# xiph/daala

Hardware: NVIDIA H100
Metric: encoder Mpixels/s on 4K YUV420 intra (higher is better)
Workload: dtype int32

## Files before the change

daala_b200/csrc/kf_engine.cu:

```cuda
#include <cuda_runtime.h>
#include <math.h>
#include <stdint.h>
#include <stdio.h>
#include <stdlib.h>
#include <string.h>

#include <algorithm>
#include <cmath>
#include <mutex>
#include <new>
#include <vector>

#include "daala_b200.h"
#include "dering_search.h"
#include "late_skip.h"
#include "lossless.h"
#include "mc_batch.h"
#include "gen/coding_order.inc"
#include "pvq_math.cuh"
#include "pvq_warp.cuh"
#include "pvq_common.cuh"

namespace daala_b200 {
namespace kf {

using namespace daala_b200::pvq;

enum Cnt {
  kNLuma = 0, kNChroma, kLumaCoefs, kChromaCoefs,
  kNItemsL = 4,
  kNItemsC = 7,
  kTotalHi = 14,
  kNHeads = 15,
  kNHeads0 = 16,
  kError = 17,
  kDepsDone = 18,
  kMcBadRef = 19,
  kMcBeyond = 20,
  kHeadLoL = 32,
  kHeadLoC = 64,
  kHeadHi = 96,
  kTailHi = 128,
  kDoneHi = 160,
  kHeadCh = 192,
  kWaiters = 224,
  kTraceN = 240,
  kCntWords = 256
};

constexpr int kTile = 1024;
constexpr int kMaxLevels = 4096;
constexpr int kLevelBins = kMaxLevels * 3;

struct Lists {
  const uint8_t* bsize;
  int bstride;
  long long bsize_pitch;
  int F, UW, UH;
  int u_row0, u_rows;
  int ntiles;
  int4* tile_sum;
  int32_t* unit_lbase;
  int32_t* unit_loff;
  daala_b200_pvq_block* luma;
  daala_b200_pvq_block* chroma;
  int32_t* dep_top;
  int32_t* dep_left;
  int32_t* succ_bottom;
  int32_t* succ_right;
  uint32_t* items_l[3];
  uint32_t* items_c[3];
  uint32_t* heads;
  uint32_t* heads0;
// ... 570 lines not shown
  }
  return kNoItem;
}

__device__ __forceinline__ void intra_band_ref(const Stage& S, int blk, int band, int coef_off, int lane) {
  const daala_b200_pvq_params& prm = S.prm;
  const int start = band_start(band);
  const int bn = band_start(band + 1) - start;
  const int r = band % 3;
  int top = -1, left = -1;
  if (band == 0 || r == 1) top = S.dep_top[blk];
  if (band == 0 || r == 2) left = S.dep_left[blk];
  if (band == 3 || band == 6) top = left = -1;
  const int32_t* ot = top >= 0 ? prm.out + prm.blocks[top].coef_off : nullptr;
  const int32_t* ol = left >= 0 ? prm.out + prm.blocks[left].coef_off : nullptr;
  bool low_from_top = false;
  if (band == 0) {
    double g1 = 0, g2 = 0;
    if (ot) { double a = __ldcg(ot + 2), bb = __ldcg(ot + 5), c = __ldcg(ot + 9); g1 += a * a; g1 += bb * bb; g1 += c * c; }
    if (ol) { double a = __ldcg(ol + 1), bb = __ldcg(ol + 4), c = __ldcg(ol + 7); g2 += a * a; g2 += bb * bb; g2 += c * c; }
    low_from_top = g1 > g2;
  }
  int32_t* vref = prm.ref + coef_off;
  for (int i = start + lane; i < start + bn; i += 32) {
    int r2, c2;
    scan_rc(i, &r2, &c2);
    int32_t p = 0;
    if (r2 == 0 && c2 > 0 && ot && (c2 >= 4 || low_from_top)) p = __ldcg(ot + i);
    if (c2 == 0 && r2 > 0 && ol && (r2 >= 4 || !low_from_top)) p = __ldcg(ol + i);
    vref[i] = p;
  }
}

template <bool kIntra>
__device__ __forceinline__ void run_item(const Stage& S, uint32_t item, int lane, int16_t* snap) {
  const daala_b200_pvq_params& prm = S.prm;
  const int blk = (int)(item >> 4), band = (int)(item & 15);
  const daala_b200_pvq_block b = prm.blocks[blk];
  const int bs = b.bs, pli = b.pli;
  const int start = band_start(band);
  const int bn = band_start(band + 1) - start;
  const size_t off = (size_t)b.coef_off + start;
  if (kIntra) intra_band_ref(S, blk, band, b.coef_off, lane);
  int qidx = bs * (bs + 1) + (band + 1) - (band + 1) / 3;
  int q = (prm.q0 * prm.pvq_qm_q4[pli][qidx]) >> 4;
  if (q < 1) q = 1;
  const int beta = (prm.use_masking && pli == 0 && bs > 0) ? kBeta15 : kBeta1;
  const int qoff = (b.xdec & 1 ? prm.qm_stride : 0) + ((((1 << (2 * bs)) - 1) << 4) / 3) + start;
  int itheta, max_theta, k;
  double skip_term;
  const bool pre = kIntra && S.pre_ev && band != 3 && band != 6;
  const int32_t* pev = pre ? S.pre_ev + (off >> 3) * kPreEvWords : nullptr;
  const int16_t* psn = pre ? S.pre_snap + 2 * off : nullptr;
  const int gain = quantise_band_warp<0>(lane, snap, S.rsqrt_tbl, prm.out + off, prm.in + off, prm.ref + off, bn, q,
                                         prm.y + off, &itheta, &max_theta, &k, beta, &skip_term, prm.is_keyframe, pli,
                                         prm.qm + qoff, prm.qm_inv + qoff, prm.pvq_norm_lambda, pev, psn);
  if (lane == 0) {
    const size_t r = (size_t)blk * 9 + band;
    prm.res_skip_term[r] = skip_term;
    short4 pk;
    pk.x = (short)gain; pk.y = (short)itheta; pk.z = (short)max_theta; pk.w = (short)k;
    reinterpret_cast<short4*>(S.res_pack)[r] = pk;
  }
}

struct ItemGeom {
  int blk, band, bn, q, beta, pli, qoff;
  size_t off;
};
__device__ __forceinline__ int band_q(const daala_b200_pvq_params& prm, const daala_b200_kf_frame_quant* fq, int frame,
                                      int pli, int qidx) {
  return fq ? (fq[frame].q0 * fq[frame].pvq_qm_q4[pli][qidx]) >> 4 : (prm.q0 * prm.pvq_qm_q4[pli][qidx]) >> 4;
}
__device__ __forceinline__ ItemGeom item_geom(const daala_b200_pvq_params& prm, uint32_t item,
                                              const daala_b200_kf_frame_quant* fq) {
  ItemGeom g;
  g.blk = (int)(item >> 4);
  g.band = (int)(item & 15);
  const daala_b200_pvq_block b = prm.blocks[g.blk];
  const int bs = b.bs;
  g.pli = b.pli;
  const int start = band_start(g.band);
  g.bn = band_start(g.band + 1) - start;
  g.off = (size_t)b.coef_off + start;
  const int qidx = bs * (bs + 1) + (g.band + 1) - (g.band + 1) / 3;
  int q = band_q(prm, fq, b.frame, g.pli, qidx);
  g.q = q < 1 ? 1 : q;
  g.beta = (prm.use_masking && g.pli == 0 && bs > 0) ? kBeta15 : kBeta1;
  g.qoff = (b.xdec & 1 ? prm.qm_stride : 0) + ((((1 << (2 * bs)) - 1) << 4) / 3) + start;
  return g;
}

template <int kPhase, bool kZeroRef, int kMode, bool kFq = false>
__global__ void __launch_bounds__(128) k_pvq_split(const __grid_constant__ Stage S, int cls, int chunk) {
  const daala_b200_pvq_params& prm = S.prm;
// ... 154 lines not shown
      if (lane == 0) {
        const int blk = (int)(item >> 4);
        if (band == 0) {
          const int nb[2] = {S.succ_bottom[blk], S.succ_right[blk]};
          for (int i = 0; i < 2; i++) {
            if (nb[i] < 0) continue;
            const int need = (S.dep_top[nb[i]] >= 0) + (S.dep_left[nb[i]] >= 0);
            if (need == 2 && atomicAdd(&S.join0[nb[i]], 1) != 1) continue;
            if (next == kNoItem) {
              next = (uint32_t)nb[i] << 4;
            } else {
              __threadfence();
              push_chain(S, nb[i], 0);
            }
          }
        } else {
          const int nb = band % 3 == 1 ? S.succ_bottom[blk] : S.succ_right[blk];
          if (nb >= 0) next = ((uint32_t)nb << 4) | band;
        }
      }
      next = __shfl_sync(0xffffffffu, next, 0);
      if (next == kNoItem) break;
      __threadfence();
      item = next;
    }
  }
}

__global__ void k_fill_rsqrt(double* tbl) {
  const int i = blockIdx.x * blockDim.x + threadIdx.x;
  if (i < kTableDoubles) pvq_fill_rsqrt_table(tbl, i);
}

enum { kBeginLuma = 1, kBeginChroma = 2 };
__global__ void k_begin_pvq(int32_t* cnt, int stages) {
  if (threadIdx.x == 0 && blockIdx.x == 0) {
    if (stages & kBeginLuma) {
      cnt[kHeadLoL] = 0;
      cnt[kHeadHi] = 0;
      cnt[kTailHi] = cnt[kNHeads0];
      cnt[kDoneHi] = 0;
      cnt[kHeadCh] = 0;
      cnt[kWaiters] = 0;
#ifdef DAALA_B200_CHAIN_TRACE
      cnt[kTraceN] = 0;
#endif
    }
    if (stages & kBeginChroma) cnt[kHeadLoC] = 0;
  }
}

template <bool kInter>
__global__ void __launch_bounds__(256) k_finish_scatter(const __grid_constant__ Stage S) {
  const daala_b200_pvq_params& prm = S.prm;
  const int n = min(S.cnt[S.n_blocks_at], S.max_blocks);
  const int lane = threadIdx.x & 31;
  const int nwarps = (gridDim.x * blockDim.x) >> 5;
  for (int blk = (blockIdx.x * blockDim.x + threadIdx.x) >> 5; blk < n; blk += nwarps) {
    const daala_b200_pvq_block b = prm.blocks[blk];
    const int ln = b.bs + 2, nn = 1 << ln;
    const int len = ln >= 5 ? 512 : 1 << (2 * ln);
    const int stride = prm.plane_stride[b.pli];
    int32_t* dst = prm.coef_plane[b.pli] + b.frame * prm.plane_frame_pitch[b.pli] + (size_t)b.y0 * stride + b.x0;
    const int32_t* src = prm.out + b.coef_off;
    if (lane == 0) {
      const int nb = num_bands(b.bs);
      double sd = 0;
      for (int i = 0; i < nb; i++) sd += prm.res_skip_term[(size_t)blk * 9 + i];
      prm.res_skip_diff[blk] = sd;
      if (!kInter) {
        prm.out[b.coef_off] = prm.in[b.coef_off];
      } else {
        int dc_quant = band_q(prm, S.fq, b.frame, b.pli, b.bs * (b.bs + 1));
        if (dc_quant < 1) dc_quant = 1;
        const int32_t r = prm.ref[b.coef_off], diff = prm.in[b.coef_off] - r;
        int qdc = 0;
        if (abs(diff) >= dc_quant * 141 / 256) {
          const int half = ((dc_quant + 1) >> 1) - 1;
          qdc = (diff + (diff < 0 ? -half : half)) / dc_quant;
        }
        prm.out[b.coef_off] = dst[0] = qdc * dc_quant + r;
// ... 467 lines not shown
  int32_t* thr[2];
  int32_t* dir;
  bool search;
  daala_b200_dering_search_batch sb;
};

enum { kEvLists, kEvForward, kEvLumaBands, kEvLumaScatter, kEvChroma, kNumEvents };

struct daala_b200_kf {
  daala_b200_kf_config cfg;
  int nhsb, nvsb, F;
  int plane_w[3], plane_h[3];
  cudaStream_t stream;
  bool own_stream;
  cudaStream_t side;
  cudaEvent_t ev[kNumEvents];
  cudaGraph_t graph;
  cudaGraphExec_t exec;
  bool captured;
  uint8_t* pixels[3];
  int32_t* coeffs[3];
  int32_t* lapped[3];
  uint8_t* pixels_out[3];
  uint8_t* pred_pixels[3];
  int32_t* pred_coeffs[3];
  uint8_t* bsize;
  int16_t *qm, *qm_inv;
  double* rsqrt_tbl;
  int16_t* sp_vec[3];
  int32_t* sp_lanes[3];
  int32_t* sp_uni[3];
  int16_t* sp_snap[3];
  int sp_slots[3];
  int16_t* lv_vec;
  int32_t* lv_lanes;
  int32_t* lv_uni;
  int16_t* lv_snap;
  int32_t* lv_bar;
  int lvl_slots, lvl_grid;
  Dering dering;
  Lists lists;
  Stage luma, chroma;
  Sym sym;
  daala_b200_frame frame;
  daala_b200_frame frame_pred;
  uint8_t* ref_pixels[3];
  int32_t* ref_slot;
  daala_b200_mv_pt* mv_grid;
  int32_t* ref_slot_next;
  int32_t* mv1_grid;
  uint32_t* mc_leaves;
  int32_t* mc_nleaves;
  daala_b200_mc_batch mc;
  uint8_t* fin_skip[2];
  int32_t* fin_dc[2];
  int32_t* dc_resid[2];
  int32_t* fin_coeffs[3];
  uint8_t* fin_pixels[3];
  uint8_t* fin_bskip[3];
  uint8_t *fin_level, *fin_coded;
  Fin fin;
  cudaGraph_t fin_graph;
  cudaGraphExec_t fin_exec;
  bool fin_captured;
  int fin_dc_limit;
  daala_b200_kf_frame_quant* fq;
// ... 185 lines not shown
    KF_CHECK(dalloc(kf, &L.items_l[c], cap_l[c]));
    KF_CHECK(dalloc(kf, &L.items_c[c], cap_c[c]));
  }
  if (kf->cfg.split_free > 0 || inter) {
    const int slots[3] = {1 << 19, 1 << 19, 3 << 15};
    for (int c = 0; c < 3; c++) {
      const int vs = c == 2 ? 128 : 32;
      kf->sp_slots[c] = slots[c];
      KF_CHECK(dalloc(kf, &kf->sp_vec[c], (size_t)slots[c] * 3 * vs));
      KF_CHECK(dalloc(kf, &kf->sp_lanes[c], (size_t)slots[c] * kCtxLaneWords * 16));
      KF_CHECK(dalloc(kf, &kf->sp_uni[c], (size_t)slots[c] * kCtxUniWords));
      KF_CHECK(dalloc(kf, &kf->sp_snap[c], (size_t)slots[c] * kMaxEvents * vs));
    }
  }
  if (kf->cfg.level_chains) {
    KF_CHECK(dalloc(kf, &L.lvl_hist, (size_t)kLevelBins));
    KF_CHECK(dalloc(kf, &L.lvl_cursor, (size_t)kLevelBins));
    KF_CHECK(dalloc(kf, &L.lvl_items, kf->chain_cap));
    L.nlevels = (kf->plane_w[0] + L.u_rows * 8) / 4 + 2;
    if (L.nlevels >= kMaxLevels) return (int)cudaErrorInvalidValue;
    kf->lvl_slots = 2048 * F;
    KF_CHECK(dalloc(kf, &kf->lv_vec, (size_t)kf->lvl_slots * 3 * 128));
    KF_CHECK(dalloc(kf, &kf->lv_lanes, (size_t)kf->lvl_slots * kCtxLaneWords * 16));
    KF_CHECK(dalloc(kf, &kf->lv_uni, (size_t)kf->lvl_slots * kCtxUniWords));
    KF_CHECK(dalloc(kf, &kf->lv_snap, (size_t)kf->lvl_slots * kMaxEvents * 128));
    KF_CHECK(dalloc(kf, &kf->lv_bar, (size_t)32));
    int per_sm = 0;
    KF_CHECK(cudaOccupancyMaxActiveBlocksPerMultiprocessor(&per_sm, k_pvq_levels, 128, 0));
    if (per_sm < 1) return (int)cudaErrorLaunchOutOfResources;
    kf->lvl_grid = per_sm * kf->sms;
  }
  {
    const int want = kf->cfg.persist_ctas_per_sm > 0 ? kf->cfg.persist_ctas_per_sm : kPersistCtas;
    int per_sm[2] = {0, 0};
    KF_CHECK(cudaFuncSetAttribute(k_pvq_persist<true>, cudaFuncAttributePreferredSharedMemoryCarveout,
                                  cudaSharedmemCarveoutMaxShared));
    KF_CHECK(cudaFuncSetAttribute(k_pvq_persist<false>, cudaFuncAttributePreferredSharedMemoryCarveout,
                                  cudaSharedmemCarveoutMaxShared));
    KF_CHECK(cudaOccupancyMaxActiveBlocksPerMultiprocessor(&per_sm[0], k_pvq_persist<true>, kPersistThreads, 0));
    KF_CHECK(cudaOccupancyMaxActiveBlocksPerMultiprocessor(&per_sm[1], k_pvq_persist<false>, kPersistThreads, 0));
    if (per_sm[0] < want || per_sm[1] < want) {
      snprintf(kf->err, sizeof(kf->err), "k_pvq_persist: %d / %d CTAs per SM resident, %d wanted", per_sm[0],
               per_sm[1], want);
      return (int)cudaErrorLaunchOutOfResources;
    }
  }
  KF_CHECK(dalloc(kf, &L.heads, inter ? 0 : kf->chain_cap));
  KF_CHECK(dalloc(kf, &L.heads_raw, inter ? 0 : kf->chain_cap));
  KF_CHECK(dalloc(kf, &L.head_bin, inter ? 0 : kf->chain_cap));
  KF_CHECK(dalloc(kf, &L.head_hist, inter ? 0 : (size_t)kLevelBins));
  KF_CHECK(dalloc(kf, &L.head_cursor, inter ? 0 : (size_t)kLevelBins));
  KF_CHECK(dalloc(kf, &L.heads0, ndep));
  KF_CHECK(dalloc(kf, &L.cnt, (size_t)kCntWords));
  kf->mc.bad_ref = L.cnt + kMcBadRef;
  kf->mc.beyond = L.cnt + kMcBeyond;

  auto setup_stage = [&](Stage& S, bool chroma) -> int {
    memset(&S, 0, sizeof(S));
    daala_b200_pvq_params& p = S.prm;
    const size_t ncoef = chroma ? luma_shard_px / 2 + 1024 : luma_shard_px + 1024;
    const size_t nblk = chroma ? L.max_chroma : L.max_luma;
    p.blocks = chroma ? L.chroma : L.luma;
    KF_CHECK(dalloc(kf, &p.in, ncoef));
    KF_CHECK(dalloc(kf, &p.ref, ncoef));
    KF_CHECK(dalloc(kf, &p.out, ncoef));
    KF_CHECK(dalloc(kf, &p.y, ncoef));
    KF_CHECK(dalloc(kf, &p.y16, ncoef));
    KF_CHECK(dalloc(kf, &p.res_skip_term, nblk * 9));
    KF_CHECK(dalloc(kf, &p.res_skip_diff, nblk));
    KF_CHECK(dalloc(kf, &p.res_flip, nblk));
    KF_CHECK(dalloc(kf, &S.res_pack, nblk * 9 * 4));
    p.res_gain = p.res_theta = p.res_max_theta = p.res_k = nullptr;
    p.res_dc = nullptr;
    if (inter) KF_CHECK(dalloc(kf, &p.res_dc, nblk));
    p.qm = kf->qm;
    p.qm_inv = kf->qm_inv;
    for (int i = 0; i < 3; i++) {
      p.coef_plane[i] = kf->coeffs[i];
// ... 8 lines not shown
    p.pvq_norm_lambda = kf->cfg.pvq_norm_lambda;
    memcpy(p.pvq_qm_q4, kf->cfg.pvq_qm_q4, sizeof(p.pvq_qm_q4));
    S.fq = kf->fq;
    for (int c = 0; c < 3; c++) S.items[c] = chroma ? L.items_c[c] : L.items_l[c];
    S.cnt = L.cnt;
    S.rsqrt_tbl = kf->rsqrt_tbl;
    for (int c = 0; c < 3; c++) {
      S.sp_vec[c] = kf->sp_vec[c];
      S.sp_lanes[c] = kf->sp_lanes[c];
      S.sp_uni[c] = kf->sp_uni[c];
      S.sp_snap[c] = kf->sp_snap[c];
      S.sp_slots[c] = kf->sp_slots[c];
      const size_t cap = chroma ? cap_c[c] : cap_l[c];
      S.sp_chunks[c] = kf->sp_slots[c] > 0 ? (int)((cap + kf->sp_slots[c] - 1) / kf->sp_slots[c]) : 0;
    }
    S.skip_lo = chroma ? 0 : kf->cfg.split_free > 1;
    S.max_waiters = getenv("DAALA_B200_MAX_WAITERS") ? atoi(getenv("DAALA_B200_MAX_WAITERS")) : kf->sms * 8;
    if (!chroma && kf->cfg.noref_prepass) {
      KF_CHECK(dalloc(kf, &S.pre_ev, (ncoef / 8 + 2) * kPreEvWords));
      KF_CHECK(dalloc(kf, &S.pre_snap, 2 * ncoef));
    }
    if (!chroma) {
      S.lvl_off = L.lvl_hist;
      S.lvl_items = L.lvl_items;
      S.nlevels = L.nlevels;
      S.lvl_slots = kf->lvl_slots;
      S.lv_vec = kf->lv_vec;
      S.lv_lanes = kf->lv_lanes;
      S.lv_uni = kf->lv_uni;
      S.lv_snap = kf->lv_snap;
      S.lv_bar = kf->lv_bar;
    }
    S.n_items_at = chroma ? kNItemsC : kNItemsL;
    S.head_lo_at = chroma ? kHeadLoC : kHeadLoL;
    S.n_blocks_at = chroma ? kNChroma : kNLuma;
    S.max_blocks = (int)nblk;
#ifdef DAALA_B200_CHAIN_TRACE
    if (!chroma && !inter) {
      S.trace_cap = (int)(luma_shard_px / 16);
      KF_CHECK(dalloc(kf, &S.trace, (size_t)S.trace_cap));
    }
#endif
    if (!chroma) {
      S.dep_top = L.dep_top;
      S.dep_left = L.dep_left;
      S.succ_bottom = L.succ_bottom;
      S.succ_right = L.succ_right;
      S.heads = L.heads;
      S.heads0 = L.heads0;
      KF_CHECK(dalloc(kf, &S.ring, inter ? 0 : kf->chain_cap));
      KF_CHECK(dalloc(kf, &S.join0, ndep));
    }
    return 0;
  };
  int rc = setup_stage(kf->luma, false);
  if (rc) return rc;
  rc = setup_stage(kf->chroma, true);
  if (rc) return rc;
  if (!inter) {
    Stage& C = kf->chroma;
    C.cfl_in = kf->luma.prm.in;
    C.cfl_out = kf->luma.prm.out;
    C.cfl_loff = L.unit_loff;
  }
  (void)luma_px;
  if (kf->cfg.inter_finish || kf->cfg.symbol_stream == 2)
    for (int c = 0; c < 2; c++) {
// ... 368 lines not shown
  }
  if (!core && (phases & DAALA_B200_KF_PVQ_CHROMA) && kf->cfg.late_skip) {
    const int rc = daala_b200_late_skip_enqueue(&kf->lsb, kf->sms * 3, s);
    if (rc) return rc;
  }
  if (!core && (phases & DAALA_B200_KF_PVQ_CHROMA) && kf->cfg.symbol_stream) enqueue_sym<true>(kf->sym, wide, s);
  if (phases & DAALA_B200_KF_INVERSE) {
    int rc = daala_b200_launch_inverse(&kf->frame, 3, s);
    if (rc) return rc;
  }
  return (int)cudaGetLastError();
}

static int enqueue_lists(daala_b200_kf* kf, cudaStream_t s) {
  const Lists& L = kf->lists;
  const int wide = kf->sms * 8;
  k_unit_tile_sums<<<L.ntiles, kTile, 0, s>>>(L);
  k_tile_scan<<<1, 1024, 0, s>>>(L);
  k_unit_emit<<<L.ntiles, kTile, 0, s>>>(L);
  const size_t nl = (size_t)L.max_luma * sizeof(int32_t);
  if (cudaMemsetAsync(L.succ_bottom, 0xff, nl, s) != cudaSuccess || cudaMemsetAsync(L.succ_right, 0xff, nl, s) != cudaSuccess)
    return (int)cudaGetLastError();
  if (L.lvl_hist && cudaMemsetAsync(L.lvl_hist, 0, sizeof(int32_t) * kLevelBins, s) != cudaSuccess) return (int)cudaGetLastError();
  if (cudaMemsetAsync(L.head_hist, 0, sizeof(int32_t) * kLevelBins, s) != cudaSuccess) return (int)cudaGetLastError();
  k_luma_deps<<<wide, 256, 0, s>>>(L);
  if (L.lvl_hist) {
    k_level_scan<<<1, 1024, 0, s>>>(L);
    k_level_scatter<<<wide, 256, 0, s>>>(L);
  }
  k_chroma_items<<<wide, 256, 0, s>>>(L);
  return 0;
}

static int enqueue_luma_bands(daala_b200_kf* kf, bool core, int begin, cudaStream_t s) {
  const int wide = kf->sms * 8;
  const int persist = kf->sms * (kf->cfg.persist_ctas_per_sm > 0 ? kf->cfg.persist_ctas_per_sm : kPersistCtas);
  if (cudaMemsetAsync(kf->luma.ring, 0xff, kf->chain_cap * sizeof(uint32_t), s) != cudaSuccess ||
      cudaMemsetAsync(kf->luma.join0, 0, (size_t)kf->luma.max_blocks * sizeof(int32_t), s) != cudaSuccess)
    return (int)cudaGetLastError();
  k_begin_pvq<<<1, 32, 0, s>>>(kf->lists.cnt, begin);
  if (!core) k_gather<kGatherLuma><<<wide, 256, 0, s>>>(kf->luma);
  if (kf->cfg.split_free > 1) enqueue_split<true>(kf, kf->luma, s);
  if (kf->luma.pre_ev) {
    k_pvq_prepass<2><<<kf->sms * 16, 128, 0, s>>>(kf->luma);
    k_pvq_prepass<1><<<kf->sms * 16, 128, 0, s>>>(kf->luma);
  }
  if (kf->cfg.level_chains) {
    if (cudaMemsetAsync(kf->lv_bar, 0, sizeof(int32_t) * 32, s) != cudaSuccess) return (int)cudaGetLastError();
    k_pvq_levels<<<kf->lvl_grid, 128, 0, s>>>(kf->luma);
  } else {
    k_pvq_persist<true><<<persist, kPersistThreads, 0, s>>>(kf->luma);
  }
  return 0;
}

static void enqueue_chroma(daala_b200_kf* kf, bool core, bool begin, cudaStream_t s) {
  const int wide = kf->sms * 8;
  if (begin) k_begin_pvq<<<1, 32, 0, s>>>(kf->lists.cnt, kBeginChroma);
  if (!core) k_gather<kGatherChroma><<<wide, 256, 0, s>>>(kf->chroma);
  if (kf->cfg.split_free > 0) enqueue_split<false>(kf, kf->chroma, s);
  else k_pvq_persist<false><<<kf->sms * (kf->cfg.persist_ctas_per_sm > 0 ? kf->cfg.persist_ctas_per_sm : kPersistCtas),
                              kPersistThreads, 0, s>>>(kf->chroma);
  if (!core) k_finish_scatter<false><<<wide, 256, 0, s>>>(kf->chroma);
}

static int kf_enqueue_step_forked(daala_b200_kf* kf) {
  cudaStream_t s = kf->stream, c = kf->side;
  const daala_b200_frame& fr = kf->cfg.dering ? kf->dering.frame : kf->frame;
  auto fork = [](cudaEvent_t e, cudaStream_t from, cudaStream_t to) {
    return cudaEventRecord(e, from) == cudaSuccess && cudaStreamWaitEvent(to, e, 0) == cudaSuccess;
  };
  if (!fork(kf->ev[kEvLists], s, c)) return (int)cudaGetLastError();
  int rc = daala_b200_launch_forward(&kf->frame, 3, c);
  if (!rc) rc = enqueue_lists(kf, s);
  if (rc) return rc;
  if (!fork(kf->ev[kEvForward], c, s)) return (int)cudaGetLastError();
  rc = enqueue_luma_bands(kf, false, kBeginLuma | kBeginChroma, s);
  if (rc) return rc;
  if (!fork(kf->ev[kEvLumaBands], s, c)) return (int)cudaGetLastError();
  enqueue_chroma(kf, false, false, c);
  k_finish_scatter<false><<<kf->sms * 128, 256, 0, s>>>(kf->luma);
  if (kf->cfg.symbol_stream) {
    if (!fork(kf->ev[kEvLumaScatter], s, c)) return (int)cudaGetLastError();
    enqueue_sym<false>(kf->sym, kf->sms * 8, c);
  }
  rc = enqueue_recon(fr, 1, 2, c);
  if (!rc) rc = enqueue_recon(fr, 0, 1, s);
  if (!rc && kf->cfg.dering) rc = enqueue_dering_luma(kf, kf->dering, s);
  if (rc) return rc;
  if (!fork(kf->ev[kEvChroma], c, s)) return (int)cudaGetLastError();
  for (int p = 1; kf->cfg.dering && p < 3; p++) {
    rc = enqueue_dering_plane(kf, kf->dering, p, s);
    if (rc) return rc;
  }
  return (int)cudaGetLastError();
}

static int kf_enqueue_step_lossless(daala_b200_kf* kf, int phases) {
  if (phases != DAALA_B200_KF_ALL) {
    snprintf(kf->err, sizeof(kf->err), "a lossless step runs whole (DAALA_B200_KF_ALL)");
    return (int)cudaErrorInvalidValue;
  }
  cudaStream_t s = kf->stream;
  const int wide = kf->sms * 8;
  if (kf->cfg.inter_mc) {
    if (cudaMemsetAsync(kf->lists.cnt + kMcBadRef, 0, 2 * sizeof(int32_t), s) != cudaSuccess) return (int)cudaGetLastError();
    int rc = daala_b200_launch_mc_leaves(&kf->mc, wide, s);
    if (!rc) rc = daala_b200_launch_mc_obmc(&kf->mc, wide, s);
    if (rc) return rc;
  }
  return daala_b200_launch_lossless(&kf->ll, s);
}

static int kf_enqueue_step(daala_b200_kf* kf, int phases) {
  if (kf->cfg.lossless) return kf_enqueue_step_lossless(kf, phases);
  if (kf->cfg.inter) return kf_enqueue_step_inter(kf, phases);
  if (phases == DAALA_B200_KF_ALL) return kf_enqueue_step_forked(kf);
  cudaStream_t s = kf->stream;
  if (phases & DAALA_B200_KF_LISTS) {
    const int rc = enqueue_lists(kf, s);
    if (rc) return rc;
  }
  if (phases & DAALA_B200_KF_FORWARD) {
    const int rc = daala_b200_launch_forward(&kf->frame, 3, s);
    if (rc) return rc;
  }
  const bool core = (phases & DAALA_B200_KF_SEARCH_ONLY) != 0;
  if (phases & DAALA_B200_KF_PVQ_LUMA) {
    const int rc = enqueue_luma_bands(kf, core, kBeginLuma, s);
    if (rc) return rc;
    if (!core) k_finish_scatter<false><<<kf->sms * 8, 256, 0, s>>>(kf->luma);
  }
  if (phases & DAALA_B200_KF_PVQ_CHROMA) {
    enqueue_chroma(kf, core, true, s);
    if (!core && kf->cfg.symbol_stream) enqueue_sym<false>(kf->sym, kf->sms * 8, s);
  }
  if (phases & DAALA_B200_KF_INVERSE) {
    int rc = kf->cfg.dering ? enqueue_dering(kf, kf->dering, s) : daala_b200_launch_inverse(&kf->frame, 3, s);
    if (rc) return rc;
  }
  return (int)cudaGetLastError();
}

static int kf_enqueue_finish(daala_b200_kf* kf) {
  cudaStream_t s = kf->stream;
  const int wide = kf->sms * 8;
  if (kf->fin_form) k_fin_unstream<<<wide, 256, 0, s>>>(kf->unstream);
  if (cudaMemsetAsync(kf->fin_coded, 0, (size_t)kf->F * kf->nhsb * kf->nvsb, s) != cudaSuccess)
    return (int)cudaGetLastError();
  k_fin_patch<<<wide, 256, 0, s>>>(kf->fin);
  k_fin_skip_map<<<wide, 256, 0, s>>>(kf->fin);
  const int rc = enqueue_dering(kf, kf->dering, s);
  if (rc) return rc;
  if (kf->fin_slot_out) k_fin_pool_store<<<dim3(wide > kf->F ? wide / kf->F : 1, 3 * kf->F), 256, 0, s>>>(kf->store);
  return (int)cudaGetLastError();
}

extern "C" {

static thread_local char g_create_err[256] = "null engine";

daala_b200_kf* daala_b200_kf_create(const daala_b200_kf_config* cfg) {
  snprintf(g_create_err, sizeof(g_create_err), "daala_b200_kf_create: invalid configuration");
  if (cfg && cfg->inter_mc && (cfg->inter_mc != 1 || cfg->inter != 1)) {
    snprintf(g_create_err, sizeof(g_create_err), "daala_b200_kf_create: inter_mc is 0 or 1, and 1 requires inter = 1");
    return nullptr;
  }
// ... 121 lines not shown
  if (kf->exec) cudaGraphExecDestroy(kf->exec);
  if (kf->graph) cudaGraphDestroy(kf->graph);
  if (kf->fin_exec) cudaGraphExecDestroy(kf->fin_exec);
  if (kf->fin_graph) cudaGraphDestroy(kf->fin_graph);
  for (void* p : kf->allocs) cudaFree(p);
  for (cudaEvent_t e : kf->ev)
    if (e) cudaEventDestroy(e);
  if (kf->side) cudaStreamDestroy(kf->side);
  if (kf->own_stream) cudaStreamDestroy(kf->stream);
  delete kf;
}

const char* daala_b200_kf_error(const daala_b200_kf* kf) { return kf ? kf->err : g_create_err; }

#ifdef DAALA_B200_CHAIN_TRACE
int daala_b200_kf_chain_trace(daala_b200_kf* kf, void** recs, int* cap) {
  if (!kf || !recs || !cap) return (int)cudaErrorInvalidValue;
  *recs = kf->luma.trace;
  *cap = kf->luma.trace_cap;
  return 0;
}
#endif

int daala_b200_kf_launches_per_step(const daala_b200_kf* kf) {
  if (!kf) return 0;
  if (kf->cfg.lossless) return (kf->cfg.inter_mc ? 2 : 0) + (kf->cfg.inter ? 1 : 2);
  auto split = [](const Stage& S) { return 3 * (S.sp_chunks[0] + S.sp_chunks[1] + S.sp_chunks[2]); };
  if (kf->cfg.inter)
    return 5 + 2 + (2 + split(kf->luma)) + (2 + split(kf->chroma)) + 2 + (kf->cfg.inter_mc ? 2 : 0) +
           (kf->cfg.symbol_stream ? 8 : 0) + (kf->cfg.late_skip ? kLateSkipLaunches : 0);
  int n = 5 + (kf->cfg.level_chains ? 2 : 0);
  n += 1;
  n += 3 + 1 + (kf->cfg.split_free > 1 ? split(kf->luma) : 0) + (kf->luma.pre_ev ? 2 : 0);
  n += 2 + (kf->cfg.split_free > 0 ? split(kf->chroma) : 1);
  n += kf->cfg.dering ? dering_launches(kf->dering, 2) : 4;
  if (kf->cfg.symbol_stream) n += 8;
  return n;
}

int daala_b200_kf_device_buffers(daala_b200_kf* kf, daala_b200_kf_buffers* out) {
  if (!kf || !out) return (int)cudaErrorInvalidValue;
  memset(out, 0, sizeof(*out));
  for (int p = 0; p < 3; p++) {
    out->pixels[p] = kf->pixels[p];
    out->coeffs[p] = kf->coeffs[p];
    out->lapped[p] = kf->lapped[p];
    out->pixels_out[p] = kf->pixels_out[p];
    out->plane_w[p] = kf->plane_w[p];
    out->plane_h[p] = kf->plane_h[p];
  }
  out->bsize = kf->bsize;
  out->counts = kf->lists.cnt;
  out->luma_blocks = kf->lists.luma;
  out->chroma_blocks = kf->lists.chroma;
  out->dep_top = kf->lists.dep_top;
  out->dep_left = kf->lists.dep_left;
  for (int c = 0; c < 3; c++) {
    out->luma_items[c] = kf->lists.items_l[c];
    out->chroma_items[c] = kf->lists.items_c[c];
  }
  out->luma_heads = kf->lists.heads;
  out->luma_heads0 = kf->lists.heads0;
  out->luma_heads_raw = kf->lists.heads_raw;
  out->luma_head_bin = kf->lists.head_bin;
  out->succ_bottom = kf->lists.succ_bottom;
  out->succ_right = kf->lists.succ_right;
  out->luma_res = kf->luma.res_pack;
// ... 532 lines not shown
```

daala_b200/csrc/pvq_warp.cuh:

```cuda
#pragma once
#include <math.h>
#include <stdint.h>

#include "pvq_math.cuh"

namespace daala_b200 {
namespace pvq {

constexpr unsigned kFull = 0xffffffffu;
constexpr int kMaxEvents = 14;
constexpr int kRsqrtEntries = 1 << 16;
constexpr int kLogEntries = 1 << 12;
constexpr int kTableDoubles = kRsqrtEntries + kLogEntries;

#ifndef DAALA_B200_PVQ_EXACT_BOUND
#define DAALA_B200_PVQ_EXACT_BOUND 4503599627370496.
#endif
#ifdef DAALA_B200_EMU_STATS
#define PVQ_WARP_STAT(i) (daala_b200_pvq_warp_stats[i]++)
#else
#define PVQ_WARP_STAT(i) ((void)0)
#endif

__device__ __forceinline__ int wsum(int v) { return __reduce_add_sync(kFull, v); }
// ... 256 lines not shown
          if (pos < 0 || t > ba) { ba = t; pos = e * 32 + l; }
        }
      }
    }
    const int src = pos & 31, slot = pos >> 5;
    int sx = v.xa[0], sy = ya[0];
#pragma unroll
    for (int e = 1; e < E; e++) if (slot == e) { sx = v.xa[e]; sy = ya[e]; }
    const int px = __shfl_sync(kFull, sx, src);
    const int py = __shfl_sync(kFull, sy, src);
    xy = xy + (double)px;
    yy = yy + 2 * py + 1;
#pragma unroll
    for (int e = 0; e < E; e++) if (e * 32 + lane == pos) ya[e]++;
  }
  *xy_out = xy;
  *yy_out = yy;
}

struct BandCtx {
  int x16[4], r16[4], xr[4];
  int32_t cg, g, gain_offset;
  int icgr, m, s;
  double best_dist, best_cost, skip_dist;
  int c_gain, c_theta, c_ts, c_k, c_cosd, c_alive, c_ev;
  int32_t c_qcg, c_qtheta;
  double c_sinprod, c_lambda, c_rate_ts;
  double e_xy, e_yy, e_xx;
  int e_sum, e_k, e_zero;
};

constexpr int kCtxLaneWords = 24;
constexpr int kCtxUniWords = 16;
constexpr int kSnapEntries = kMaxEvents * kMaxN + 3 * kMaxN + 2 * (kCtxLaneWords * 16 + kCtxUniWords);

#ifdef __CUDACC__
__device__ __forceinline__ void ctx_sync() { __syncwarp(); }
#else
inline void ctx_sync() {}
#endif

__device__ __forceinline__ void ctx_put_d(int32_t* lanes, int w, int lane, double v) {
  lanes[w * 16 + lane] = __double2loint(v);
  lanes[(w + 1) * 16 + lane] = __double2hiint(v);
}
__device__ __forceinline__ double ctx_get_d(const int32_t* lanes, int w, int lane) {
  return __hiloint2double(lanes[(w + 1) * 16 + lane], lanes[w * 16 + lane]);
}

__device__ __forceinline__ void band_ctx_store_setup(int lane, const BandCtx& B, int n, int16_t* vec, int vstride,
                                                     int32_t* lanes, int32_t* uni) {
#pragma unroll
  for (int e = 0; e < 4; e++) {
    const int j = e * 32 + lane;
    if (j < n) {
      vec[j] = (int16_t)B.x16[e];
      vec[vstride + j] = (int16_t)B.r16[e];
      vec[2 * vstride + j] = (int16_t)B.xr[e];
    }
  }
  if (lane < 16) {
    lanes[0 * 16 + lane] = B.c_gain;
    lanes[1 * 16 + lane] = B.c_theta;
    lanes[2 * 16 + lane] = B.c_ts;
    lanes[3 * 16 + lane] = B.c_k;
    lanes[4 * 16 + lane] = B.c_cosd;
    lanes[5 * 16 + lane] = B.c_alive;
// ... 527 lines not shown
  *vk = best_k;
  *skip_term = skip_dist - best_dist;
  if (is_keyframe) return noref ? qg : (qg < icgr ? -2 * (qg - icgr) - 1 : (qg < 2 * icgr ? 2 * (qg - icgr) : qg - 1));
  {
    const int a = qg + 1, b = icgr + 1;
    return noref ? qg - 1 : (a < b ? -2 * (a - b) - 1 : (a < 2 * b ? 2 * (a - b) : a - 1));
  }
}

constexpr int kPreEvWords = 20;
__device__ __forceinline__ void band_noref_export(int lane, const BandCtx& B, int n, const int16_t* snap,
                                                  int snap_stride, int32_t* pre_ev, int16_t* pre_snap) {
  const int cev = (lane == 12 || lane == 13) ? B.c_ev : -1;
  const int nev = wmax(cev) + 1;
  if (lane == 12 || lane == 13) pre_ev[lane - 12] = B.c_ev;
  if (lane < nev) {
    int32_t* r = pre_ev + 2 + lane * 9;
    r[0] = __double2loint(B.e_xy); r[1] = __double2hiint(B.e_xy);
    r[2] = __double2loint(B.e_yy); r[3] = __double2hiint(B.e_yy);
    r[4] = __double2loint(B.e_xx); r[5] = __double2hiint(B.e_xx);
    r[6] = B.e_sum; r[7] = B.e_k; r[8] = B.e_zero;
  }
  for (int ev = 0; ev < nev; ev++)
    for (int j = lane; j < n; j += 32) pre_snap[ev * n + j] = snap[ev * snap_stride + j];
}

template <int kMode = 0>
__device__ __forceinline__ int quantise_band_warp(int lane, int16_t* snap, const double* rsq, int32_t* out, const int32_t* x0,
                                                  const int32_t* r0, int n, int q0, int32_t* yout, int* itheta,
                                                  int* max_theta, int* vk, int beta, double* skip_term, int is_keyframe,
                                                  int pli, const int16_t* qm, const int16_t* qm_inv,
                                                  double pvq_norm_lambda, const int32_t* pre_ev = nullptr,
                                                  const int16_t* pre_snap = nullptr) {
  int16_t* vec = snap + kMaxEvents * kMaxN;
  int32_t* lanes = reinterpret_cast<int32_t*>(vec + 3 * kMaxN);
  int32_t* uni = lanes + kCtxLaneWords * 16;
  {
    BandCtx B;
    band_setup<kMode>(lane, B, x0, r0, n, q0, beta, is_keyframe, pli, qm, pvq_norm_lambda, rsq);
    ctx_sync();
    band_ctx_store_setup(lane, B, n, vec, kMaxN, lanes, uni);
  }
  ctx_sync();
  {
    BandCtx B;
    band_ctx_load_search(lane, B, n, vec, kMaxN, lanes);
    band_search<kMode>(lane, B, n, snap, kMaxN, rsq, pre_ev, pre_snap);
    band_ctx_store_search(lane, B, lanes);
  }
  ctx_sync();
  BandCtx B;
  band_ctx_load_finish(lane, B, n, vec, kMaxN, lanes, uni);
  return band_finish<kMode>(lane, B, snap, kMaxN, out, r0, n, q0, yout, itheta, max_theta, vk, beta, skip_term, is_keyframe, pli,
                     qm_inv, pvq_norm_lambda);
}

}
}
```

Baseline: 2451.

## Replace chroma persistent PVQ kernel with size-specialized warp-per-CTA chroma kernels

Chroma PVQ no longer runs through the persistent chain-scheduled kernel. Two specialised kernels now handle it: one for the large-band item lists (mode 2) and one for small bands (mode 1). The mode 1 kernel uses a compact 32-wide shared-scratch stride so that more single-warp CTAs fit per SM. The chroma head counter reset is dropped, which trades dynamic scheduling for flat grid-stride loops with higher occupancy and adds one more launch to the chroma path.

Result: no change. 2449 (median of 6 runs) (-0.1%).

```diff
diff --git a/daala_b200/csrc/kf_engine.cu b/daala_b200/csrc/kf_engine.cu
--- a/daala_b200/csrc/kf_engine.cu
+++ b/daala_b200/csrc/kf_engine.cu
@@ -38,7 +38,6 @@
   kMcBadRef = 19,
   kMcBeyond = 20,
   kHeadLoL = 32,
-  kHeadLoC = 64,
   kHeadHi = 96,
   kTailHi = 128,
   kDoneHi = 160,
@@ -675,7 +674,7 @@
   }
 }
 
-template <bool kIntra>
+template <bool kIntra, int kMode = 0>
 __device__ __forceinline__ void run_item(const Stage& S, uint32_t item, int lane, int16_t* snap) {
   const daala_b200_pvq_params& prm = S.prm;
   const int blk = (int)(item >> 4), band = (int)(item & 15);
@@ -695,7 +694,7 @@
   const bool pre = kIntra && S.pre_ev && band != 3 && band != 6;
   const int32_t* pev = pre ? S.pre_ev + (off >> 3) * kPreEvWords : nullptr;
   const int16_t* psn = pre ? S.pre_snap + 2 * off : nullptr;
-  const int gain = quantise_band_warp<0>(lane, snap, S.rsqrt_tbl, prm.out + off, prm.in + off, prm.ref + off, bn, q,
+  const int gain = quantise_band_warp<kMode>(lane, snap, S.rsqrt_tbl, prm.out + off, prm.in + off, prm.ref + off, bn, q,
                                          prm.y + off, &itheta, &max_theta, &k, beta, &skip_term, prm.is_keyframe, pli,
                                          prm.qm + qoff, prm.qm_inv + qoff, prm.pvq_norm_lambda, pev, psn);
   if (lane == 0) {
@@ -704,6 +703,25 @@
     short4 pk;
     pk.x = (short)gain; pk.y = (short)itheta; pk.z = (short)max_theta; pk.w = (short)k;
     reinterpret_cast<short4*>(S.res_pack)[r] = pk;
+  }
+}
+
+constexpr int kChromaThreads = 32;
+template <int kMode>
+constexpr int kChromaCtas = kMode == 1 ? 24 : 16;
+static_assert(kChromaCtas<1> * (kBandScratchEntries<1> * (int)sizeof(int16_t) + 1024) <= 228 * 1024 &&
+              kChromaCtas<2> * (kBandScratchEntries<2> * (int)sizeof(int16_t) + 1024) <= 228 * 1024,
+              "k_pvq_chroma's shared scratch does not fit kChromaCtas CTAs per SM");
+template <int kMode>
+__global__ void __launch_bounds__(kChromaThreads, kChromaCtas<kMode>) k_pvq_chroma(const __grid_constant__ Stage S) {
+  __shared__ __align__(16) int16_t snap[kBandScratchEntries<kMode>];
+  const int lane = threadIdx.x & 31;
+  const int hi = kMode == 2 ? 2 : 1;
+  const int nwarps = (gridDim.x * blockDim.x) >> 5;
+  for (int i = (blockIdx.x * blockDim.x + threadIdx.x) >> 5;
+       i < S.cnt[S.n_items_at + hi] + (kMode == 1 ? S.cnt[S.n_items_at] : 0); i += nwarps) {
+    const int n_hi = S.cnt[S.n_items_at + hi];
+    run_item<false, kMode>(S, i < n_hi ? S.items[hi][i] : S.items[0][i - n_hi], lane, snap);
   }
 }
 
@@ -924,21 +942,17 @@
   if (i < kTableDoubles) pvq_fill_rsqrt_table(tbl, i);
 }
 
-enum { kBeginLuma = 1, kBeginChroma = 2 };
-__global__ void k_begin_pvq(int32_t* cnt, int stages) {
+__global__ void k_begin_pvq(int32_t* cnt) {
   if (threadIdx.x == 0 && blockIdx.x == 0) {
-    if (stages & kBeginLuma) {
-      cnt[kHeadLoL] = 0;
-      cnt[kHeadHi] = 0;
-      cnt[kTailHi] = cnt[kNHeads0];
-      cnt[kDoneHi] = 0;
-      cnt[kHeadCh] = 0;
-      cnt[kWaiters] = 0;
+    cnt[kHeadLoL] = 0;
+    cnt[kHeadHi] = 0;
+    cnt[kTailHi] = cnt[kNHeads0];
+    cnt[kDoneHi] = 0;
+    cnt[kHeadCh] = 0;
+    cnt[kWaiters] = 0;
 #ifdef DAALA_B200_CHAIN_TRACE
-      cnt[kTraceN] = 0;
+    cnt[kTraceN] = 0;
 #endif
-    }
-    if (stages & kBeginChroma) cnt[kHeadLoC] = 0;
   }
 }
 
@@ -1472,6 +1486,7 @@
   int32_t* sp_uni[3];
   int16_t* sp_snap[3];
   int sp_slots[3];
+  int chroma_grid[2];
   int16_t* lv_vec;
   int32_t* lv_lanes;
   int32_t* lv_uni;
@@ -1723,18 +1738,30 @@
   }
   {
     const int want = kf->cfg.persist_ctas_per_sm > 0 ? kf->cfg.persist_ctas_per_sm : kPersistCtas;
-    int per_sm[2] = {0, 0};
+    int per_sm = 0;
     KF_CHECK(cudaFuncSetAttribute(k_pvq_persist<true>, cudaFuncAttributePreferredSharedMemoryCarveout,
                                   cudaSharedmemCarveoutMaxShared));
-    KF_CHECK(cudaFuncSetAttribute(k_pvq_persist<false>, cudaFuncAttributePreferredSharedMemoryCarveout,
+    KF_CHECK(cudaOccupancyMaxActiveBlocksPerMultiprocessor(&per_sm, k_pvq_persist<true>, kPersistThreads, 0));
+    if (per_sm < want) {
+      snprintf(kf->err, sizeof(kf->err), "k_pvq_persist: %d CTAs per SM resident, %d wanted", per_sm, want);
+      return (int)cudaErrorLaunchOutOfResources;
+    }
+  }
+  if (!inter) {
+    int per_sm[2] = {0, 0};
+    KF_CHECK(cudaFuncSetAttribute(k_pvq_chroma<1>, cudaFuncAttributePreferredSharedMemoryCarveout,
                                   cudaSharedmemCarveoutMaxShared));
-    KF_CHECK(cudaOccupancyMaxActiveBlocksPerMultiprocessor(&per_sm[0], k_pvq_persist<true>, kPersistThreads, 0));
-    KF_CHECK(cudaOccupancyMaxActiveBlocksPerMultiprocessor(&per_sm[1], k_pvq_persist<false>, kPersistThreads, 0));
-    if (per_sm[0] < want || per_sm[1] < want) {
-      snprintf(kf->err, sizeof(kf->err), "k_pvq_persist: %d / %d CTAs per SM resident, %d wanted", per_sm[0],
-               per_sm[1], want);
+    KF_CHECK(cudaFuncSetAttribute(k_pvq_chroma<2>, cudaFuncAttributePreferredSharedMemoryCarveout,
+                                  cudaSharedmemCarveoutMaxShared));
+    KF_CHECK(cudaOccupancyMaxActiveBlocksPerMultiprocessor(&per_sm[0], k_pvq_chroma<1>, kChromaThreads, 0));
+    KF_CHECK(cudaOccupancyMaxActiveBlocksPerMultiprocessor(&per_sm[1], k_pvq_chroma<2>, kChromaThreads, 0));
+    if (per_sm[0] < kChromaCtas<1> || per_sm[1] < kChromaCtas<2>) {
+      snprintf(kf->err, sizeof(kf->err), "k_pvq_chroma: %d / %d CTAs per SM resident, %d / %d wanted", per_sm[0],
+               per_sm[1], kChromaCtas<1>, kChromaCtas<2>);
       return (int)cudaErrorLaunchOutOfResources;
     }
+    kf->chroma_grid[0] = kChromaCtas<1> * kf->sms;
+    kf->chroma_grid[1] = kChromaCtas<2> * kf->sms;
   }
   KF_CHECK(dalloc(kf, &L.heads, inter ? 0 : kf->chain_cap));
   KF_CHECK(dalloc(kf, &L.heads_raw, inter ? 0 : kf->chain_cap));
@@ -1809,7 +1836,7 @@
       S.lv_bar = kf->lv_bar;
     }
     S.n_items_at = chroma ? kNItemsC : kNItemsL;
-    S.head_lo_at = chroma ? kHeadLoC : kHeadLoL;
+    S.head_lo_at = kHeadLoL;
     S.n_blocks_at = chroma ? kNChroma : kNLuma;
     S.max_blocks = (int)nblk;
 #ifdef DAALA_B200_CHAIN_TRACE
@@ -2244,13 +2271,13 @@
   return 0;
 }
 
-static int enqueue_luma_bands(daala_b200_kf* kf, bool core, int begin, cudaStream_t s) {
+static int enqueue_luma_bands(daala_b200_kf* kf, bool core, cudaStream_t s) {
   const int wide = kf->sms * 8;
   const int persist = kf->sms * (kf->cfg.persist_ctas_per_sm > 0 ? kf->cfg.persist_ctas_per_sm : kPersistCtas);
   if (cudaMemsetAsync(kf->luma.ring, 0xff, kf->chain_cap * sizeof(uint32_t), s) != cudaSuccess ||
       cudaMemsetAsync(kf->luma.join0, 0, (size_t)kf->luma.max_blocks * sizeof(int32_t), s) != cudaSuccess)
     return (int)cudaGetLastError();
-  k_begin_pvq<<<1, 32, 0, s>>>(kf->lists.cnt, begin);
+  k_begin_pvq<<<1, 32, 0, s>>>(kf->lists.cnt);
   if (!core) k_gather<kGatherLuma><<<wide, 256, 0, s>>>(kf->luma);
   if (kf->cfg.split_free > 1) enqueue_split<true>(kf, kf->luma, s);
   if (kf->luma.pre_ev) {
@@ -2266,13 +2293,15 @@
   return 0;
 }
 
-static void enqueue_chroma(daala_b200_kf* kf, bool core, bool begin, cudaStream_t s) {
+static void enqueue_chroma(daala_b200_kf* kf, bool core, cudaStream_t s) {
   const int wide = kf->sms * 8;
-  if (begin) k_begin_pvq<<<1, 32, 0, s>>>(kf->lists.cnt, kBeginChroma);
   if (!core) k_gather<kGatherChroma><<<wide, 256, 0, s>>>(kf->chroma);
-  if (kf->cfg.split_free > 0) enqueue_split<false>(kf, kf->chroma, s);
-  else k_pvq_persist<false><<<kf->sms * (kf->cfg.persist_ctas_per_sm > 0 ? kf->cfg.persist_ctas_per_sm : kPersistCtas),
-                              kPersistThreads, 0, s>>>(kf->chroma);
+  if (kf->cfg.split_free > 0) {
+    enqueue_split<false>(kf, kf->chroma, s);
+  } else {
+    k_pvq_chroma<2><<<kf->chroma_grid[1], kChromaThreads, 0, s>>>(kf->chroma);
+    k_pvq_chroma<1><<<kf->chroma_grid[0], kChromaThreads, 0, s>>>(kf->chroma);
+  }
   if (!core) k_finish_scatter<false><<<wide, 256, 0, s>>>(kf->chroma);
 }
 
@@ -2287,10 +2316,10 @@
   if (!rc) rc = enqueue_lists(kf, s);
   if (rc) return rc;
   if (!fork(kf->ev[kEvForward], c, s)) return (int)cudaGetLastError();
-  rc = enqueue_luma_bands(kf, false, kBeginLuma | kBeginChroma, s);
+  rc = enqueue_luma_bands(kf, false, s);
   if (rc) return rc;
   if (!fork(kf->ev[kEvLumaBands], s, c)) return (int)cudaGetLastError();
-  enqueue_chroma(kf, false, false, c);
+  enqueue_chroma(kf, false, c);
   k_finish_scatter<false><<<kf->sms * 128, 256, 0, s>>>(kf->luma);
   if (kf->cfg.symbol_stream) {
     if (!fork(kf->ev[kEvLumaScatter], s, c)) return (int)cudaGetLastError();
@@ -2339,12 +2368,12 @@
   }
   const bool core = (phases & DAALA_B200_KF_SEARCH_ONLY) != 0;
   if (phases & DAALA_B200_KF_PVQ_LUMA) {
-    const int rc = enqueue_luma_bands(kf, core, kBeginLuma, s);
+    const int rc = enqueue_luma_bands(kf, core, s);
     if (rc) return rc;
     if (!core) k_finish_scatter<false><<<kf->sms * 8, 256, 0, s>>>(kf->luma);
   }
   if (phases & DAALA_B200_KF_PVQ_CHROMA) {
-    enqueue_chroma(kf, core, true, s);
+    enqueue_chroma(kf, core, s);
     if (!core && kf->cfg.symbol_stream) enqueue_sym<false>(kf->sym, kf->sms * 8, s);
   }
   if (phases & DAALA_B200_KF_INVERSE) {
@@ -2532,7 +2561,7 @@
   int n = 5 + (kf->cfg.level_chains ? 2 : 0);
   n += 1;
   n += 3 + 1 + (kf->cfg.split_free > 1 ? split(kf->luma) : 0) + (kf->luma.pre_ev ? 2 : 0);
-  n += 2 + (kf->cfg.split_free > 0 ? split(kf->chroma) : 1);
+  n += 2 + (kf->cfg.split_free > 0 ? split(kf->chroma) : 2);
   n += kf->cfg.dering ? dering_launches(kf->dering, 2) : 4;
   if (kf->cfg.symbol_stream) n += 8;
   return n;
diff --git a/daala_b200/csrc/pvq_warp.cuh b/daala_b200/csrc/pvq_warp.cuh
--- a/daala_b200/csrc/pvq_warp.cuh
+++ b/daala_b200/csrc/pvq_warp.cuh
@@ -312,7 +312,11 @@
 
 constexpr int kCtxLaneWords = 24;
 constexpr int kCtxUniWords = 16;
-constexpr int kSnapEntries = kMaxEvents * kMaxN + 3 * kMaxN + 2 * (kCtxLaneWords * 16 + kCtxUniWords);
+template <int kMode>
+constexpr int kBandVstride = kMode == 1 ? 32 : kMaxN;
+template <int kMode>
+constexpr int kBandScratchEntries = (kMaxEvents + 3) * kBandVstride<kMode> + 2 * (kCtxLaneWords * 16 + kCtxUniWords);
+constexpr int kSnapEntries = kBandScratchEntries<0>;
 
 #ifdef __CUDACC__
 __device__ __forceinline__ void ctx_sync() { __syncwarp(); }
@@ -906,26 +910,27 @@
                                                   int pli, const int16_t* qm, const int16_t* qm_inv,
                                                   double pvq_norm_lambda, const int32_t* pre_ev = nullptr,
                                                   const int16_t* pre_snap = nullptr) {
-  int16_t* vec = snap + kMaxEvents * kMaxN;
-  int32_t* lanes = reinterpret_cast<int32_t*>(vec + 3 * kMaxN);
+  constexpr int vs = kBandVstride<kMode>;
+  int16_t* vec = snap + kMaxEvents * vs;
+  int32_t* lanes = reinterpret_cast<int32_t*>(vec + 3 * vs);
   int32_t* uni = lanes + kCtxLaneWords * 16;
   {
     BandCtx B;
     band_setup<kMode>(lane, B, x0, r0, n, q0, beta, is_keyframe, pli, qm, pvq_norm_lambda, rsq);
     ctx_sync();
-    band_ctx_store_setup(lane, B, n, vec, kMaxN, lanes, uni);
+    band_ctx_store_setup(lane, B, n, vec, vs, lanes, uni);
   }
   ctx_sync();
   {
     BandCtx B;
-    band_ctx_load_search(lane, B, n, vec, kMaxN, lanes);
-    band_search<kMode>(lane, B, n, snap, kMaxN, rsq, pre_ev, pre_snap);
+    band_ctx_load_search(lane, B, n, vec, vs, lanes);
+    band_search<kMode>(lane, B, n, snap, vs, rsq, pre_ev, pre_snap);
     band_ctx_store_search(lane, B, lanes);
   }
   ctx_sync();
   BandCtx B;
-  band_ctx_load_finish(lane, B, n, vec, kMaxN, lanes, uni);
-  return band_finish<kMode>(lane, B, snap, kMaxN, out, r0, n, q0, yout, itheta, max_theta, vk, beta, skip_term, is_keyframe, pli,
+  band_ctx_load_finish(lane, B, n, vec, vs, lanes, uni);
+  return band_finish<kMode>(lane, B, snap, vs, out, r0, n, q0, yout, itheta, max_theta, vk, beta, skip_term, is_keyframe, pli,
                      qm_inv, pvq_norm_lambda);
 }
 
```
